# SanPen/CSparse3

Hardware: AMD Instinct MI355X
Metric: numeric-LU + lsolve/usolve nnz/s on 50k power-grid Jacobian (higher is better)
Workload: dtype f64; 1 GPU; configs[2]: synthetic banded power-grid Jacobian 50000x50000, 501330 nnz, LU refactor + 1-RHS solve per step, one matrix per GPU; n=50000, nnz_a=501330, nnz_l=696852, nnz_u=696852, rhs=1, supernodes=5970, levels=12, max_front=469, ordering=amd(A+A')

## Files before the change

csparse3_amd/csrc/cs3_internal.hpp:

```cpp
#pragma once
#include <cstdint>
#include <string>
#include <vector>

#include "../../include/csparse3_amd.h"

namespace cs3 {

using i32 = int32_t;
using i64 = int64_t;

void set_error(const std::string &msg);

void symmetrized_pattern(i64 n, const i32 *Ap, const i32 *Ai,
                         std::vector<i64> &Cp, std::vector<i32> &Ci);
void amd_order(i64 n, const std::vector<i64> &Cp, const std::vector<i32> &Ci,
               std::vector<i32> &perm);

i64 match_scale(i64 n, const i32 *Ap, const i32 *Ai, const double *Ax, i32 *rowperm, double *dr, double *dc);

void etree_upper(i64 n, const i32 *Ap, const i32 *Ai, i32 *parent);
void tree_postorder(i64 n, const i32 *parent, i32 *post);
void cholesky_counts(i64 n, const i32 *Ap, const i32 *Ai, const i32 *parent,
                     const i32 *post, i32 *colcount);

enum FrontClass : int { FC_R16 = 0, FC_R32 = 1, FC_R64 = 2, FC_LDS = 3, FC_BIG = 4, FC_IL = 5, FC_SUB = 6, FC_COUNT = 7 };

enum SolveKind : int {
    SK_SMALL = 0,
    SK_WAVE = 1,
    SK_BLOCK = 2,
    SK_BIG = 3,
    SK_IL = 4,
    SK_SUB = 5
};

struct LaunchGroup {
    int level;
    int cls;
    i32 first, count;
    i32 max_r;
    i32 max_w;
    i32 n16 = 0;
};

constexpr i32 SUB_RMAX = 32;

struct SubFront {
    i32 lpan, upan;
    i32 cb;
    i32 cv;
    i32 c0, r, w;
    i32 a_begin, a_count;
    i32 child_begin, child_count;
    i32 rel;
    i32 st;
    i32 u_sj;
    i32 parent;
    i32 arena;
};

struct SubTask {
    i32 front0, nfronts;
    i32 lvl0, nlevels;
    i32 rel0, nrel;
    i32 child0, nchild;
};

struct SubForest {
    i32 ntasks = 0;
    i32 max_fronts = 0, max_levels = 0, max_rel = 0, max_child = 0;
    i32 max_arena = 0;
    i32 max_varena = 0;
    i32 max_r = 0;
    bool empty() const { return ntasks == 0; }
};
// ... 86 lines not shown
```

csparse3_amd/csrc/kernels.hip:

```cpp
#include <hip/hip_runtime.h>


#include <stdint.h>

#include <algorithm>
#include <cstdlib>

#include "cs3_device.hpp"
#include "cs3_devfn.hpp"

namespace cs3 {

hipError_t set_withhold_handover(int on)
{
    hipError_t e = hipMemcpyToSymbol(HIP_SYMBOL(g_withhold_handover), &on, sizeof(int));
    return e != hipSuccess ? e : set_withhold_handover_forest(on);
}

typedef double double4_t __attribute__((ext_vector_type(4)));

__device__ __forceinline__ double *il_lane_base(const IlView &il, long long m)
{
    return il.base + (m >> 6) * 64 * il.len + (m & 63);
}
// ... 1141 lines not shown
{
    const long long t_start = tbuf ? (long long) __builtin_amdgcn_s_memtime() : 0;
#define CS3_BSTAMP(p) do { if (tbuf && kb == 64 && blockIdx.x == 1 && blockIdx.y == 0 && threadIdx.x == 0) \
        tbuf[(long long) (first + blockIdx.z / batch) * 8 + (p)] = (long long) __builtin_amdgcn_s_memtime() - t_start; } while (0)
#define CS3_BSTAMP_ROW(p) do { if (tbuf && kb == 64 && blockIdx.x == 0 && blockIdx.y == 1 && threadIdx.x == 0) \
        tbuf[(long long) (first + blockIdx.z / batch) * 8 + (p)] = (long long) __builtin_amdgcn_s_memtime() - t_start; } while (0)
    __shared__ double As[BIG_NB][64 + 1];
    __shared__ double Bs[BIG_NB][64 + 1];
    __shared__ double Ad[BIG_NB][BIG_NB + 1];
    __shared__ double Bd[BIG_NB][BIG_NB + 1];
    __shared__ double D[BIG_NB][BIG_NB + 1];
    __shared__ double T[64][BIG_NB + 1];
    __shared__ int pair_ready[2];
    if (threadIdx.x < 2) pair_ready[threadIdx.x] = 0;
    const FrontDesc d = fdesc[first + blockIdx.z / batch];
    const int bz = blockIdx.z % batch;
    const int r = d.r, w = d.w;
    const int nblk = (w + BIG_NB - 1) / BIG_NB;
    if (kb > nblk * BIG_NB) return;
    const bool has_panel = kb < w;
    const int ke = has_panel ? min(kb + BIG_NB, w) : w, bw = ke - kb;
    const int kp = kb - BIG_NB, pw = min(kb, w) - kp;
    double *F = pool_all + (long long) bz * pool_stride + d.lpan;
    double *dbuf = dbuf_all + (long long) bz * dbuf_stride + d.dbuf;
    const long long ld = r;
    const int tid = threadIdx.x;
    const int bi = blockIdx.x, bj = blockIdx.y;
    const int nsl = (r - ke + 63) / 64;
    if (bi > nsl || bj > nsl) return;
    if (KIND == CS3_CHOLESKY && bi < bj) return;
    if (kb > 0 && bi == 0 && bj == 0) {
        const int blk = kb / BIG_NB - 1;
        const int k0 = blk * BIG_NB, cw = min(BIG_NB, w - k0);
        for (int e = tid; e < cw * cw; e += 256) {
            const int i = e % cw, j = e / cw;
            if (KIND == CS3_LU || i >= j) F[(k0 + i) + (k0 + j) * ld] = dbuf[blk * (BIG_NB * BIG_NB) + i + j * BIG_NB];
        }
    }
    if (!has_panel && (bi == 0 || bj == 0)) return;
    const int row0 = (bi == 0) ? kb : ke + (bi - 1) * 64, nrow = (bi == 0) ? bw : min(64, r - row0);
    const int col0 = (bj == 0) ? kb : ke + (bj - 1) * 64, ncol = (bj == 0) ? bw : min(64, r - col0);
    const bool needs_d = has_panel && (bi == 0 || bj == 0);

    auto raw = [](const double *__restrict__ p, long long off, bool ok) -> double { return p[ok ? off : 0]; };
    double ra[8], rb[8], rad[4], rbd[4];
    if (kb > 0) {
#pragma unroll
        for (int q = 0; q < 8; ++q) {
            const int e = tid + 256 * q;
            { const int i = e % 64, k = e / 64; ra[q] = raw(F, (row0 + i) + (long long) (kp + k) * ld, k < pw && i < nrow); }
            if (KIND == CS3_LU) { const int k = e % BIG_NB, j = e / BIG_NB; rb[q] = raw(F, (kp + k) + (long long) (col0 + j) * ld, k < pw && j < ncol); }
            else { const int j = e % 64, k = e / 64; rb[q] = raw(F, (col0 + j) + (long long) (kp + k) * ld, k < pw && j < ncol); }
        }
#pragma unroll
        for (int q = 0; q < 4; ++q) {
            const int e = tid + 256 * q;
            { const int i = e % BIG_NB, k = e / BIG_NB; rad[q] = raw(F, (kb + i) + (long long) (kp + k) * ld, needs_d && k < pw && i < bw); }
            if (KIND == CS3_LU) { const int k = e % BIG_NB, j = e / BIG_NB; rbd[q] = raw(F, (kp + k) + (long long) (kb + j) * ld, needs_d && k < pw && j < bw); }
            else { const int j = e % BIG_NB, k = e / BIG_NB; rbd[q] = raw(F, (kb + j) + (long long) (kp + k) * ld, needs_d && k < pw && j < bw); }
        }
    }
    const int wv = tid >> 6, mi = tid & 15, mq = (tid >> 4) & 3;
    const int ti = 16 * wv + mi;
    double4_t acc[4];
#pragma unroll
    for (int cb = 0; cb < 4; ++cb)
#pragma unroll
// ... 71 lines not shown
        D[dr][j] = (dr < bw && j < bw) ? dacc[v] : (dr == j ? 1.0 : 0.0);
    }
    if (bi > 0) {
#pragma unroll
        for (int cb = 0; cb < 2; ++cb)
#pragma unroll
            for (int v = 0; v < 4; ++v) T[ti][16 * cb + mq + 4 * v] = acc[cb][v];
    } else if (bj > 0 && wv < 2) {
#pragma unroll
        for (int cb = 0; cb < 4; ++cb)
#pragma unroll
            for (int v = 0; v < 4; ++v) T[16 * cb + mq + 4 * v][ti] = acc[cb][v];
    }
    __syncthreads();
    CS3_BSTAMP(3);
    const int lane = tid & 63, half = (tid >> 6) & 1, part = tid >> 7, li = lane & 31;
    const bool stacked = lane >= 32;
    const bool row_tile = (bi == 0 && bj > 0);
    const bool diag_tile = (bi == 0 && bj == 0);
    if (diag_tile && half == 1) return;
    constexpr int HC = PAIR_NC;
    const int cbase = HC * part;
    double e[HC];
#pragma unroll
    for (int j = 0; j < HC; ++j) {
        const double dv = row_tile ? D[cbase + j][li] : D[li][cbase + j];
        const double tv = T[32 * half + li][cbase + j];
        e[j] = stacked ? (diag_tile ? 0.0 : tv) : dv;
    }
    eliminate_pair<KIND>(e, part, row_tile, (half == 0) ? &As[0][0] : &Bs[0][0], &pair_ready[half], status);
    CS3_BSTAMP(4);
    CS3_BSTAMP_ROW(6);
    if (diag_tile) {
        double *db = dbuf + (long long) (kb / BIG_NB) * (BIG_NB * BIG_NB);
        if (lane < bw) {
#pragma unroll
            for (int jj = 0; jj < HC; ++jj) {
                const int j = cbase + jj;
                if (j < bw) {
                    const double v = e[jj];
                    if (KIND == CS3_LU) {
                        if (lane > j) { if (!(fabs(v) <= inv_tol)) flag_column(status, d.c0 + kb + j); }
                        else if (lane == j) { if (!(fabs(v) > 0.0) || !(fabs(v) < 1.0e300)) flag_column(status, d.c0 + kb + j); }
                    } else if (lane == j) {
                        if (!(v > 0.0)) flag_column(status, d.c0 + kb + j);
                    }
                    db[lane + j * BIG_NB] = v;
                }
            }
        }
        return;
    }
    const int tr = 32 * half + li;
    if (stacked) {
        if (!row_tile) {
            if (tr < nrow) {
#pragma unroll
                for (int cc = 0; cc < HC; ++cc) {
                    const int c = cbase + cc;
                    if (c < bw) {
                        if (KIND == CS3_LU && !(fabs(e[cc]) <= inv_tol)) flag_column(status, d.c0 + kb + c);
                        F[(row0 + tr) + (long long) (kb + c) * ld] = e[cc];
                    }
                }
            }
        } else if (tr < ncol) {
#pragma unroll
            for (int cc = 0; cc < HC; ++cc) {
                const int c = cbase + cc;
                if (c < bw) F[(kb + c) + (long long) (col0 + tr) * ld] = e[cc];
            }
        }
    }
    CS3_BSTAMP(5);
    CS3_BSTAMP_ROW(7);
#undef CS3_BSTAMP
#undef CS3_BSTAMP_ROW
}


// ... 783 lines not shown
    const int b = blockIdx.y / nrhs, rhs = blockIdx.y % nrhs;
    const int r = d.r, w = d.w, nb = r - w;
    const double *pool = pool_all + (long long) b * pool_stride;
    const double *X = X_all + (long long) b * x_stride;
    double *v = bigv_all + ((long long) b * nrhs + rhs) * bv_size + d.bv;
    const int *st = st_idx + d.st;
    const int tid = threadIdx.x;
    for (int j = tid; j < nb; j += 256) v2[j] = X[(long long) st[w + j] * nrhs + rhs];
    __syncthreads();
    const double *L = pool + d.lpan;
    const double *U = pool + d.upan;
    for (int i = blockIdx.x * 256 + tid; i < w; i += gridDim.x * 256) {
        double acc = 0.0;
        for (int j0 = 0; j0 < nb; j0 += 16) {
            double u[16];
#pragma unroll
            for (int j = 0; j < 16; ++j) {
                const int jj = j0 + j;
                const long long off = (KIND == CS3_LU) ? (long long) i * d.u_sk + (long long) jj * d.u_sj
                                                       : (long long) (w + jj) + (long long) i * r;
                u[j] = load_if((KIND == CS3_LU) ? U : L, off, jj < nb);
            }
#pragma unroll
            for (int j = 0; j < 16; ++j) acc += u[j] * v2[j0 + j < nb ? j0 + j : 0];
        }
        v[i] = X[(long long) (d.c0 + i) * nrhs + rhs] - acc;
    }
}

template <int KIND, int CW>
__global__ void __launch_bounds__(256)
k_bwd_big_step(const SolveDesc *__restrict__ sd, int first, int chunk_from_right,
               const double *__restrict__ pool_all, double *__restrict__ X_all, double *__restrict__ bigv_all,
               int nrhs, long long pool_stride, long long x_stride, long long bv_size)
{
    constexpr int SC = CW / 4;
    __shared__ double y[BIG_CW];
    __shared__ double cpl[64];
    __shared__ double part[4][64];
    const SolveDesc d = sd[first + blockIdx.z];
    const int r = d.r, w = d.w;
    const int nchunk = (w + CW - 1) / CW;
    const int c = nchunk - 1 - chunk_from_right;
    if (c < 0) return;
    const int kb = c * CW, bw = min(CW, w - kb);
    const int bwa = min(SOLVE_BW, bw), bwb = bw - bwa;
    const int nsl = (kb + 63) / 64;
    if ((int) blockIdx.x > 0 && (int) blockIdx.x >= nsl) return;
    const int b = blockIdx.y / nrhs, rhs = blockIdx.y % nrhs;
    const double *L = pool_all + (long long) b * pool_stride + d.lpan;
    double *v = bigv_all + ((long long) b * nrhs + rhs) * bv_size + d.bv;
    const int tid = threadIdx.x, lane = tid & 63, wv = tid >> 6;
    const int row = blockIdx.x * 64 + lane;
    double us[SC];
#pragma unroll
    for (int j = 0; j < SC; ++j) {
        const int jj = wv * SC + j;
        const long long off = (KIND == CS3_LU) ? (long long) row + (long long) (kb + jj) * r
                                               : (long long) (kb + jj) + (long long) row * r;
        us[j] = load_if(L, off, row < kb && jj < bw);
    }
    if (wv == 0) {
        if (bwb > 0) {
            BlockTriangle<KIND, false> tb;
            tb.load(L, r, kb + SOLVE_BW, bwb);
            const double vi = tb.solve(load_if(v, kb + SOLVE_BW + lane, lane < bwb), bwb);
            if (lane < bwb) y[SOLVE_BW + lane] = vi;
        }
        __syncthreads();
        __syncthreads();
    } else if (wv == 1) {
        BlockTriangle<KIND, false> ta;
        ta.load(L, r, kb, bwa);
        __syncthreads();
        __syncthreads();
        const double vi = ta.solve(cpl[lane], bwa);
        if (lane < bwa) y[lane] = vi;
    } else if (wv == 2) {
        double tm[SOLVE_BW];
#pragma unroll
        for (int j = 0; j < SOLVE_BW; ++j) {
            const long long i = kb + lane, k = kb + SOLVE_BW + j;
            const long long off = (KIND == CS3_LU) ? i + k * r : k + i * r;
            tm[j] = load_if(L, off, lane < bwa && j < bwb);
        }
        double vi = load_if(v, kb + lane, lane < bwa);
        __syncthreads();
#pragma unroll
        for (int j = 0; j < SOLVE_BW; ++j) vi -= tm[j] * ((j < bwb) ? y[SOLVE_BW + j] : 0.0);
        cpl[lane] = vi;
        __syncthreads();
    } else {
        __syncthreads();
        __syncthreads();
    }
    __syncthreads();
    if (blockIdx.x == 0 && tid < bw)
        X_all[(long long) b * x_stride + (long long) (d.c0 + kb + tid) * nrhs + rhs] = y[tid];
    double acc = 0.0;
#pragma unroll
    for (int j = 0; j < SC; ++j) {
        const int jj = wv * SC + j;
        acc += us[j] * y[jj < bw ? jj : 0];
    }
    part[wv][lane] = acc;
    __syncthreads();
    if (tid < 64 && row < kb)
        v[row] -= ((part[0][tid] + part[1][tid]) + part[2][tid]) + part[3][tid];
}

constexpr int IL_KB = 4;
constexpr int IL_T = 8;
constexpr int IL_TJ = 4;
constexpr int IL_NONE = INT32_MIN;
constexpr int IL_AV = 32;

template <int KIND>
__global__ void __launch_bounds__(64)
k_front_il(const FrontDesc *__restrict__ fdesc, int first, const int *__restrict__ pairs,
           const double *__restrict__ ax_all, long long nnz_a, IlView il,
           const double *__restrict__ pool_pm_all, long long pm_stride, int batch, double inv_tol, int *status)
{
    const FrontDesc d = fdesc[first + blockIdx.x];
    const int lane = threadIdx.x;
    const long long m = (long long) blockIdx.y * 64 + lane;
    const bool live = m < batch;
    const long long mm = live ? m : (long long) blockIdx.y * 64;
    double *G = il.base + (long long) blockIdx.y * 64 * il.len + lane;
    const double *P = pool_pm_all + mm * pm_stride;
    const double *ax = ax_all + mm * nnz_a;
    const int r = d.r, w = d.w;
    double *F = G + d.lpan * 64;
#define EL(i, j) F[((long long) (i) + (long long) (j) * r) * 64]

    {
        const int np = d.a_count;
        const int *pr = pairs + 2 * d.a_begin;
        int cur = -1;
        double acc = 0.0;
        int ptg_n = pr[2 * (lane < min(64, np) ? lane : 0)], psr_n = pr[2 * (lane < min(64, np) ? lane : 0) + 1];
        for (int base = 0; base < np; base += 64) {
// ... 868 lines not shown

__global__ void __launch_bounds__(256)
k_restack_values(long long nnz, const int *__restrict__ map, long long na, long long nb, long long nc,
                 const double *__restrict__ Ax, const double *__restrict__ Bx, const double *__restrict__ Cx,
                 const double *__restrict__ Dx, double *__restrict__ Px)
{
    for (long long p = (long long) blockIdx.x * blockDim.x + threadIdx.x; p < nnz; p += (long long) gridDim.x * blockDim.x) {
        const long long s = map[p];
        Px[p] = (s < na) ? Ax[s] : (s < na + nb) ? Bx[s - na] : (s < na + nb + nc) ? Cx[s - na - nb] : Dx[s - na - nb - nc];
    }
}

hipError_t launch_restack_values(long long nnz, const int *map, long long na, long long nb, long long nc, const double *Ax,
                                 const double *Bx, const double *Cx, const double *Dx, double *Px, hipStream_t st)
{
    if (nnz == 0) return hipSuccess;
    hipLaunchKernelGGL(k_restack_values, dim3((unsigned) std::min<long long>((nnz + 255) / 256, 4096)), dim3(256), 0, st, nnz, map,
                       na, nb, nc, Ax, Bx, Cx, Dx, Px);
    return hipGetLastError();
}

constexpr int RHS_LANES_MIN = 16;
#define CS3_LAUNCH_CHECK() do { hipError_t e_ = hipGetLastError(); if (e_ != hipSuccess) return e_; } while (0)

static int grid_for(long long work, int block, int cap = 4096)
{
    long long g = (work + block - 1) / block;
    if (g < 1) g = 1;
    if (g > cap) g = cap;
    return (int) g;
}

static int big_group_blocks(const LaunchGroup &g) { return (g.max_w + BIG_NB - 1) / BIG_NB; }

static hipError_t launch_big_gather(const DeviceFactor &D, const LaunchGroup &g, hipStream_t st)
{
    const int gx = std::max(1, std::min(64, (g.max_r + 7) / 8));
    hipLaunchKernelGGL(k_big_gather, dim3(gx, (unsigned) D.batch, g.count), dim3(256), 0, st, D.fdesc, g.first, D.kind,
                       AsmLists{D.fa_tgt, D.fa_src, D.ch_tab, D.rel_idx}, D.ax, D.pool_pm, D.nnz_a, D.pm_stride, IlView{D.pool_il, D.il_len});
    CS3_LAUNCH_CHECK();
    return hipSuccess;
}

template <int KIND>
static hipError_t launch_big_block(const DeviceFactor &D, const LaunchGroup &g, int blk, double inv_tol, hipStream_t st)
{
    const unsigned batch = (unsigned) D.batch;
    const int kb = blk * BIG_NB;
    const int start = std::max(1, kb - BIG_NB + 1);
    const int rem = g.max_r - std::min(start, g.max_r);
    const int tiles = 1 + (rem + 63) / 64;
    hipLaunchKernelGGL((k_big_step<KIND>), dim3(tiles, tiles, g.count * batch), dim3(256), 0, st, D.fdesc,
                       g.first, kb, D.pool_pm, D.pm_stride, D.dbuf, D.dbuf_size, inv_tol, D.status, (int) batch, D.tbuf);
    CS3_LAUNCH_CHECK();
    return hipSuccess;
}

static int wg_panel_ld(const LaunchGroup &g) { return (g.max_r + 1) | 1; }
constexpr int WG_NB = 16;
static int wg_nb() { return WG_NB; }
static size_t wg_lds_bytes(int kind, const LaunchGroup &g)
{
    return ((size_t) wg_nb() * 33 + (size_t) (kind == CS3_LU ? 2 : 1) * wg_nb() * wg_panel_ld(g) +
            (kind == CS3_LU ? 0 : (size_t) 16 * (size_t) g.max_w)) * sizeof(double);
}
bool big_group_in_one_workgroup(int kind, long long batch, const LaunchGroup &g)
{
    static const long long min_batch = getenv("CS3_WG_MIN_BATCH") ? atoll(getenv("CS3_WG_MIN_BATCH")) : 48;
    return g.cls == FC_BIG && batch >= min_batch && wg_lds_bytes(kind, g) <= 150 * 1024;
}

template <int KIND>
static hipError_t launch_front_group(const DeviceFactor &D, const SweepCall &call, const LaunchGroup &g, double inv_tol, hipStream_t st)
{
    const unsigned batch = (unsigned) D.batch;
    if (g.cls == FC_SUB) return launch_sub_factor(D, call, inv_tol, st);
    if (big_group_in_one_workgroup(KIND, D.batch, g)) {
        hipLaunchKernelGGL((k_front_wg<KIND, WG_NB>), dim3((unsigned) g.count, batch), dim3(512), wg_lds_bytes(KIND, g), st, D.fdesc,
                           g.first, AsmLists{D.fa_tgt, D.fa_src, D.ch_tab, D.rel_idx}, D.ax, D.pool_pm, D.nnz_a, D.pm_stride,
                           IlView{D.pool_il, D.il_len}, inv_tol, D.status, wg_panel_ld(g), D.tbuf);
        CS3_LAUNCH_CHECK();
        return hipSuccess;
    }
    if (g.cls == FC_IL) {
        hipLaunchKernelGGL((k_front_il<KIND>), dim3((unsigned) g.count, (unsigned) D.ngroups), dim3(64), 0, st, D.fdesc, g.first,
                           D.ila_pairs, D.ax, D.nnz_a, IlView{D.pool_il, D.il_len}, D.pool_pm, D.pm_stride, (int) D.batch,
                           inv_tol, D.status);
        CS3_LAUNCH_CHECK();
        return hipSuccess;
    }
    if (g.cls == FC_BIG) {
        hipError_t e = launch_big_gather(D, g, st);
        for (int blk = 0; e == hipSuccess && blk <= big_group_blocks(g); ++blk) e = launch_big_block<KIND>(D, g, blk, inv_tol, st);
        return e;
    }
    dim3 grid((unsigned) g.count, batch);
    const size_t ld = (size_t) (g.max_r | 1);
    const bool packed = KIND == CS3_CHOLESKY && g.max_w <= 32;
    const size_t lds = ((packed ? (size_t) g.max_r * (size_t) (g.max_r + 1) / 2 : ld * (size_t) g.max_r) + 4 * (size_t) g.max_r + 6) * sizeof(double);
#define CS3_FRONT_ARGS D.fdesc, g.first, AsmLists{D.fa_tgt, D.fa_src, D.ch_tab, D.rel_idx}, D.ax, D.pool_pm, D.nnz_a, D.pm_stride, IlView{D.pool_il, D.il_len}, inv_tol, D.status, D.tbuf
    switch (g.cls) {
    case FC_R16:
    case FC_R32:
        hipLaunchKernelGGL((k_front_wave<KIND>), grid, dim3(64), lds, st, CS3_FRONT_ARGS); break;
    case FC_R64: {
        const unsigned threads = (D.batch >= 16 && g.max_w <= 32) ? 128 : 256;
        hipLaunchKernelGGL((k_front_mix<KIND>), grid, dim3(threads), lds, st, CS3_FRONT_ARGS); break;
    }
    default:
        const size_t blds = ((KIND == CS3_LU) ? ld * (size_t) g.max_r : (size_t) g.max_r * (size_t) (g.max_r + 1) / 2) * sizeof(double) + 16;
        if (KIND == CS3_CHOLESKY && D.batch >= 16)
            hipLaunchKernelGGL((k_front_block<CS3_CHOLESKY, 16, 4>), grid, dim3(256), blds, st, CS3_FRONT_ARGS);
        else
            hipLaunchKernelGGL((k_front_block<KIND, 16>), grid, dim3(512), blds, st, CS3_FRONT_ARGS);
        break;
    }
#undef CS3_FRONT_ARGS
    CS3_LAUNCH_CHECK();
    return hipSuccess;
}

__global__ void __launch_bounds__(256) k_poison_lds(int words)
{
    extern __shared__ __attribute__((aligned(16))) double pz[];
    for (int i = threadIdx.x; i < words; i += 256) pz[i] = __longlong_as_double(0x7ff8dead0000beefll);
    __syncthreads();
// ... 148 lines not shown
    pl.nchunk = (g.max_w + pl.cw - 1) / pl.cw;
    pl.slices = std::max(1, (g.max_r + 63) / 64);
    return pl;
}

static hipError_t launch_fwd_big_pre(const DeviceFactor &D, const SweepCall &call, const LaunchGroup &g, double *X, int nrhs, hipStream_t st)
{
    const BigSweepPlan pl = big_sweep_plan(D, g, nrhs);
    hipLaunchKernelGGL(k_fwd_big_gather, dim3(1, pl.by, g.count), dim3(256), 0, st, call.sd, g.first, D.fasm_src,
                       D.fasm_tgt, D.flong_src, D.cv, X, D.bigv, nrhs, D.cv_size * (long long) nrhs, D.n * (long long) nrhs, D.bv_size);
    CS3_LAUNCH_CHECK();
    return hipSuccess;
}

template <int KIND>
static hipError_t launch_fwd_big_chunk(const DeviceFactor &D, const SweepCall &call, const LaunchGroup &g, double *X, int nrhs, int c,
                                       hipStream_t st)
{
    const BigSweepPlan pl = big_sweep_plan(D, g, nrhs);
    const long long xs = D.n * (long long) nrhs, cvs = D.cv_size * (long long) nrhs;
    if (pl.wide)
        hipLaunchKernelGGL((k_fwd_big_step<KIND, BIG_CW>), dim3(pl.slices, pl.by, g.count), dim3(256), 0, st, call.sd,
                           g.first, c * pl.cw, D.pool_pm, D.cv, X, D.bigv, nrhs, D.pm_stride, cvs, xs, D.bv_size);
    else if (pl.multi)
        hipLaunchKernelGGL((k_fwd_big_step_multi<KIND>), dim3(pl.slices, pl.by_multi, g.count), dim3(256), 0, st, call.sd,
                           g.first, c * pl.cw, D.pool_pm, D.cv, X, D.bigv, nrhs, D.pm_stride, cvs, xs, D.bv_size);
    else
        hipLaunchKernelGGL((k_fwd_big_step<KIND, SOLVE_BW>), dim3(pl.slices, pl.by, g.count), dim3(256), 0, st, call.sd,
                           g.first, c * pl.cw, D.pool_pm, D.cv, X, D.bigv, nrhs, D.pm_stride, cvs, xs, D.bv_size);
    CS3_LAUNCH_CHECK();
    return hipSuccess;
}

template <int KIND>
static hipError_t launch_bwd_big_pre(const DeviceFactor &D, const SweepCall &call, const LaunchGroup &g, double *X, int nrhs, hipStream_t st)
{
    const BigSweepPlan pl = big_sweep_plan(D, g, nrhs);
    const size_t lds = (size_t) std::max(1, g.max_r) * sizeof(double);
    hipLaunchKernelGGL((k_bwd_big_init<KIND>), dim3(2, pl.by, g.count), dim3(256), lds, st, call.sd, g.first,
                       D.st_idx, D.pool_pm, X, D.bigv, nrhs, D.pm_stride, D.n * (long long) nrhs, D.bv_size);
    CS3_LAUNCH_CHECK();
    return hipSuccess;
}

template <int KIND>
static hipError_t launch_bwd_big_chunk(const DeviceFactor &D, const SweepCall &call, const LaunchGroup &g, double *X, int nrhs, int c,
                                       hipStream_t st)
{
    const BigSweepPlan pl = big_sweep_plan(D, g, nrhs);
    const long long xs = D.n * (long long) nrhs;
    if (pl.wide)
        hipLaunchKernelGGL((k_bwd_big_step<KIND, BIG_CW>), dim3(pl.slices, pl.by, g.count), dim3(256), 0, st, call.sd,
                           g.first, c, D.pool_pm, X, D.bigv, nrhs, D.pm_stride, xs, D.bv_size);
    else if (pl.multi)
        hipLaunchKernelGGL((k_bwd_big_step_multi<KIND>), dim3(pl.slices, pl.by_multi, g.count), dim3(256), 0, st, call.sd,
                           g.first, c, D.pool_pm, X, D.bigv, nrhs, D.pm_stride, xs, D.bv_size);
    else
        hipLaunchKernelGGL((k_bwd_big_step<KIND, SOLVE_BW>), dim3(pl.slices, pl.by, g.count), dim3(256), 0, st, call.sd,
                           g.first, c, D.pool_pm, X, D.bigv, nrhs, D.pm_stride, xs, D.bv_size);
    CS3_LAUNCH_CHECK();
    return hipSuccess;
}


template <int KIND>
static hipError_t launch_inv_tasks(const DeviceFactor &D, int t0, int t1, hipStream_t st)
{
    if (t1 <= t0) return hipSuccess;
    hipLaunchKernelGGL((k_inv_diag<KIND>), dim3((unsigned) (t1 - t0), (unsigned) D.batch), dim3(256), 0, st, D.sdesc, D.inv_tasks, t0,
                       D.pool_pm, D.pm_stride, D.dinv, D.dinv_size);
    CS3_LAUNCH_CHECK();
    return hipSuccess;
}

static bool gemm_sweeps_on()
{
    static const bool on = !(getenv("CS3_NO_GEMM_SWEEPS") && getenv("CS3_NO_GEMM_SWEEPS")[0] == '1');
    return on;
}

bool permutation_can_fuse(const DeviceFactor &D, int nrhs)
{
    constexpr int min_rhs = 256;
    return gemm_sweeps_on() && nrhs >= std::max(min_rhs, RHS_LANES_MIN) && D.il_len == 0;
}

hipError_t launch_diag_inverses(const DeviceFactor &D, hipStream_t st)
{
    return with_kind(D.kind, [&](auto K) { return launch_inv_tasks<K>(D, 0, D.n_inv_tasks, st); });
}

template <int KIND>
// ... 106 lines not shown
                                   D.pool_pm, X, nrhs, D.pm_stride, xs);
        }
    } else if (g.cls == SK_BIG) {
        const BigSweepPlan pl = big_sweep_plan(D, g, nrhs);
        hipError_t e = forward ? launch_fwd_big_pre(D, call, g, X, nrhs, st) : launch_bwd_big_pre<KIND>(D, call, g, X, nrhs, st);
        for (int c = 0; e == hipSuccess && c < pl.nchunk; ++c)
            e = forward ? launch_fwd_big_chunk<KIND>(D, call, g, X, nrhs, c, st) : launch_bwd_big_chunk<KIND>(D, call, g, X, nrhs, c, st);
        return e;
    } else {
        dim3 grid((unsigned) g.count, (unsigned) D.batch, (unsigned) nrhs);
        const size_t lds = (size_t) (g.max_r + 1 + SOLVE_BW) * sizeof(double);
        if (forward)
            hipLaunchKernelGGL((k_fwd_blk<KIND>), grid, dim3(256), lds, st, call.sd, g.first, D.fasm_src,
                               D.fasm_tgt, D.flong_src, D.pool_pm, D.cv, X, nrhs, D.pm_stride, cvs, xs);
        else
            hipLaunchKernelGGL((k_bwd_blk<KIND>), grid, dim3(256), lds, st, call.sd, g.first, D.st_idx,
                               D.pool_pm, X, nrhs, D.pm_stride, xs);
    }
    CS3_LAUNCH_CHECK();
    return hipSuccess;
}

static int promote_max()
{
    return 16;
}

static void absorb_small_group(std::vector<LaunchGroup> &out, const LaunchGroup &g, int small_cls, int wg_cls)
{
    if (!out.empty() && out.back().level == g.level && out.back().cls == small_cls && g.cls == wg_cls &&
        out.back().count <= promote_max() && out.back().first + out.back().count == g.first) {
        LaunchGroup &m = out.back();
        m.cls = wg_cls; m.count += g.count;
        m.max_r = std::max(m.max_r, g.max_r); m.max_w = std::max(m.max_w, g.max_w);
        m.n16 = 0;
    } else {
        out.push_back(g);
    }
}

static std::vector<LaunchGroup> sweep_groups(const std::vector<LaunchGroup> &groups, int nrhs, long long batch)
{
    if (nrhs >= RHS_LANES_MIN) return groups;
    std::vector<LaunchGroup> merged, out;
    for (const LaunchGroup &g : groups) {
        if (!merged.empty() && merged.back().level == g.level && merged.back().cls == SK_SMALL && g.cls == SK_WAVE &&
            merged.back().first + merged.back().count == g.first) {
            LaunchGroup &m = merged.back();
            m.cls = SK_WAVE; m.count += g.count;
            m.max_r = std::max(m.max_r, g.max_r); m.max_w = std::max(m.max_w, g.max_w);
        } else {
            merged.push_back(g);
        }
    }
    if (batch != 1) return merged;
    for (const LaunchGroup &g : merged) absorb_small_group(out, g, SK_WAVE, SK_BLOCK);
    return out;
}

static std::vector<LaunchGroup> factor_groups(const DeviceFactor &D, const std::vector<LaunchGroup> &groups)
{
    if (D.batch != 1) return groups;
    std::vector<LaunchGroup> out;
    for (const LaunchGroup &g : groups) absorb_small_group(out, g, FC_R64, FC_LDS);
    return out;
}

hipError_t launch_solve_levels(const DeviceFactor &D, const SweepCall &call, double *X, int nrhs, bool forward, hipStream_t st, ForkJoin &fj)
{
    const std::vector<LaunchGroup> groups = sweep_groups(*call.groups, nrhs, D.batch);
    fj.rewind();
    const bool solve_parallel = nrhs >= 512;
    auto launch = [&](const LaunchGroup &g, hipStream_t s) {
        return with_sweep_kind(D.kind, call.trans, [&](auto K) { return launch_solve_group<K>(D, call, g, X, nrhs, forward, s); });
    };
    if (forward) {
        for (size_t g0 = 0; g0 < groups.size(); ) {
            const size_t g1 = level_edge(groups, g0, true);
            hipError_t e = run_level(groups, g0, g1, st, fj, solve_parallel, launch);
            if (e != hipSuccess) return e;
            g0 = g1;
        }
    } else {
// ... 63 lines not shown
            const int level = fgroups[f0].level;
            const size_t f1 = level_edge(fgroups, f0, true);
            e = run_level(fgroups, f0, f1, st, fj, true, [&](const LaunchGroup &g, hipStream_t s2) {
                return with_kind(D.kind, [&](auto K) { return launch_front_group<K>(D, call, g, inv_tol, s2); });
            });
            if (e != hipSuccess) return e;
            if ((e = flush()) != hipSuccess) return e;
            if ((e = fj.event(&pending)) != hipSuccess) return e;
            if ((e = hipEventRecord(pending, st)) != hipSuccess) return e;
            pending_level = level;
            f0 = f1;
        }
        if ((e = flush()) != hipSuccess) return e;
        hipEvent_t done;
        if ((e = fj.event(&done)) != hipSuccess) return e;
        if ((e = hipEventRecord(done, fj.aux)) != hipSuccess) return e;
        return hipStreamWaitEvent(st, done, 0);
    }
    const LaunchGroup *rootf = nullptr, *roots = nullptr;
    if (nrhs < RHS_LANES_MIN && nlevels >= 2 && fork_level == nlevels - 2) {
        int nf = 0, ns = 0;
        for (const LaunchGroup &g : fgroups) if (g.level == nlevels - 1) { ++nf; rootf = &g; }
        for (const LaunchGroup &g : sgroups) if (g.level == nlevels - 1) { ++ns; roots = &g; }
        if (nf != 1 || ns != 1 || rootf->cls != FC_BIG || roots->cls != SK_BIG || rootf->count != roots->count)
            rootf = roots = nullptr;
    }
    hipEvent_t swept = nullptr, ready_deferred = nullptr;
    int root_rest = 0;
    for (size_t f0 = 0; f0 < fgroups.size(); ) {
        const int level = fgroups[f0].level;
        const size_t f1 = level_edge(fgroups, f0, true);
        if (rootf && level == nlevels - 1) {
            const BigSweepPlan pl = big_sweep_plan(D, *roots, nrhs);
            const int nblk = big_group_blocks(*rootf), cwb = pl.cw / BIG_NB;
            if ((e = launch_big_gather(D, *rootf, st)) != hipSuccess) return e;
            int k = 0;
            while (k < pl.nchunk && (k + 1) * cwb <= nblk && nblk - (k + 1) * cwb >= k + 2) ++k;
            hipEvent_t home = nullptr;
            bool side_started = false;
            auto start_side = [&]() -> hipError_t {
                side_started = true;
                if (ready_deferred) {
                    hipError_t se;
                    if ((se = hipStreamWaitEvent(fj.aux, ready_deferred, 0)) != hipSuccess) return se;
                    if ((se = sweep(0, fork_level, fj.aux)) != hipSuccess) return se;
                }
                return launch_fwd_big_pre(D, call, *roots, X, nrhs, fj.aux);
            };
            auto release = [&]() -> hipError_t {
                hipError_t se;
                if ((se = hipStreamWaitEvent(fj.aux, home, 0)) != hipSuccess) return se;
                for (int c = 0; c < k; ++c) {
                    se = with_sweep_kind(D.kind, call.trans,
                                         [&](auto K) { return launch_fwd_big_chunk<K>(D, call, *roots, X, nrhs, c, fj.aux); });
                    if (se != hipSuccess) return se;
                }
                home = nullptr;
                return hipSuccess;
            };
            for (int blk = 0; blk <= nblk; ++blk) {
                e = with_kind(D.kind, [&](auto K) { return launch_big_block<K>(D, *rootf, blk, inv_tol, st); });
                if (e != hipSuccess) return e;
                if (!side_started && (e = start_side()) != hipSuccess) return e;
                if (home && (e = release()) != hipSuccess) return e;
                if (k > 0 && blk == k * cwb) {
                    if ((e = fj.event(&home)) != hipSuccess) return e;
                    if ((e = hipEventRecord(home, st)) != hipSuccess) return e;
                }
            }
            if (home && (e = release()) != hipSuccess) return e;
            root_rest = k;
            if ((e = fj.event(&swept)) != hipSuccess) return e;
            if ((e = hipEventRecord(swept, fj.aux)) != hipSuccess) return e;
            f0 = f1;
            continue;
        }
        e = run_level(fgroups, f0, f1, st, fj, true, [&](const LaunchGroup &g, hipStream_t s) {
            return with_kind(D.kind, [&](auto K) { return launch_front_group<K>(D, call, g, inv_tol, s); });
        });
        if (e != hipSuccess) return e;
        if (ready_deferred && !rootf) {
            if ((e = hipStreamWaitEvent(fj.aux, ready_deferred, 0)) != hipSuccess) return e;
            if ((e = sweep(0, fork_level, fj.aux)) != hipSuccess) return e;
            if ((e = fj.event(&swept)) != hipSuccess) return e;
            if ((e = hipEventRecord(swept, fj.aux)) != hipSuccess) return e;
            ready_deferred = nullptr;
        }
        if (level == fork_level) {
            hipEvent_t ready;
            if ((e = fj.event(&ready)) != hipSuccess) return e;
            if ((e = hipEventRecord(ready, st)) != hipSuccess) return e;
            ready_deferred = ready;
        }
// ... 68 lines not shown
```

csparse3_amd/csrc/symbolic.cpp:

```cpp
#include <algorithm>
#include <chrono>
#include <cstdlib>
#include <numeric>
#include <stdexcept>

#include "cs3_internal.hpp"
#include <cstdio>
#include <cstdlib>

namespace cs3 {

void etree_upper(i64 n, const i32 *Ap, const i32 *Ai, i32 *parent)
{
    std::vector<i32> anc(n, -1);
    for (i64 k = 0; k < n; ++k) {
        parent[k] = -1;
        for (i64 p = Ap[k]; p < Ap[k + 1]; ++p) {
            for (i32 i = Ai[p]; i != -1 && i < k; ) {
                i32 up = anc[i];
                anc[i] = (i32) k;
                if (up == -1) parent[i] = (i32) k;
                i = up;
            }
        }
// ... 738 lines not shown
            {
                const i64 r = order_r(s);
                size_t a = 0;
                for (i64 tj = 0; tj < r; ++tj)
                    for (i64 ti = (kind == CS3_CHOLESKY ? tj : 0); ti < r; ++ti) {
                        const i32 t = (i32) (ti + tj * r);
                        if (a < items.size() && items[a].tgt < t) throw std::runtime_error("analyze: source outside the stored part of a front");
                        if (a == items.size() || items[a].tgt != t) { S.ila_pairs.push_back(t); S.ila_pairs.push_back(IL_ZERO); }
                        for (; a < items.size() && items[a].tgt == t; ++a) { S.ila_pairs.push_back(t); S.ila_pairs.push_back(items[a].src); }
                    }
                if (a != items.size()) throw std::runtime_error("analyze: source outside the stored part of a front");
                while ((S.ila_pairs.size() / 2) % 16) { S.ila_pairs.push_back(-1); S.ila_pairs.push_back(IL_ZERO); }
            }
            S.ila_ptr[s + 1] = (i64) (S.ila_pairs.size() / 2);
        }
    }
    if (has_forest) fill_forest(S, fa_ptr, fa_item);

    tick("9. assembly lists");
    S.sched.resize(ns);
    std::iota(S.sched.begin(), S.sched.end(), 0);
    std::stable_sort(S.sched.begin(), S.sched.end(), [&](i32 a, i32 b) {
        if (S.sn_tlevel[a] != S.sn_tlevel[b]) return S.sn_tlevel[a] < S.sn_tlevel[b];
        return S.sn_class[a] < S.sn_class[b];
    });
    S.groups.clear();
    for (i32 t = 0; t < ns; ) {
        i32 s = S.sched[t];
        LaunchGroup g{S.sn_tlevel[s], S.sn_class[s], t, 0, 0, 0, 0};
        while (t < ns && S.sn_tlevel[S.sched[t]] == g.level && S.sn_class[S.sched[t]] == g.cls) {
            const i32 f = S.sched[t];
            g.max_r = std::max<i32>(g.max_r, (i32) order_r(f));
            g.max_w = std::max<i32>(g.max_w, (i32) width(f));
            ++t;
        }
        g.count = t - g.first;
        S.groups.push_back(g);
    }
    tick("10. launch groups");
    std::vector<i32> cs_count;
    std::vector<Item> cs_out;
    auto sort_by_row = [&](std::vector<Item> &items, i64 r) {
        cs_count.assign((size_t) r + 1, 0);
        for (const Item &it : items) ++cs_count[(size_t) it.tgt + 1];
        for (i64 t = 0; t < r; ++t) cs_count[(size_t) t + 1] += cs_count[(size_t) t];
        cs_out.resize(items.size());
        for (const Item &it : items) cs_out[(size_t) cs_count[(size_t) it.tgt]++] = it;
        items.swap(cs_out);
    };
    S.fasm_ptr.assign(ns + 1, 0);
    S.fasm_src.clear(); S.fasm_tgt.clear(); S.flong_src.clear();
    {
        std::vector<Item> items;
        for (i32 s = 0; s < ns; ++s) {
            items.clear();
            const i64 w = width(s);
            for (i64 i = 0; i < w; ++i) items.push_back(Item{(i32) i, (i32) ~(S.sn_ptr[s] + i)});
            for (i32 cp = S.child_ptr[s]; cp < S.child_ptr[s + 1]; ++cp) {
                const i32 c = S.child_idx[cp];
                const i64 nbc = order_r(c) - width(c);
                const i32 *rel = S.rel_idx.data() + S.rel_ptr[c];
                for (i64 ii = 0; ii < nbc; ++ii) items.push_back(Item{rel[ii], (i32) (S.cv_off[c] + ii)});
            }
            sort_by_row(items, order_r(s));
            emit_runs(items, S.fasm_tgt, S.fasm_src, S.flong_src);
            S.fasm_ptr[s + 1] = (i64) S.fasm_tgt.size();
// ... 42 lines not shown
                for (const Item &it : items) S.sl_src[base + (size_t) (fill[(size_t) it.tgt]++ * stride + it.tgt)] = it.src;
                S.sl_rounds[s] = rounds;
            }
            S.rl_ptr[s + 1] = (i64) (S.rl_pairs.size() / 2);
            S.sl_ptr[s + 1] = (i64) S.sl_src.size();
        }
    }
    S.ssched.resize(ns);
    std::iota(S.ssched.begin(), S.ssched.end(), 0);
    std::stable_sort(S.ssched.begin(), S.ssched.end(), [&](i32 a, i32 b) {
        if (S.sn_level[a] != S.sn_level[b]) return S.sn_level[a] < S.sn_level[b];
        if (solve_kind(a) != solve_kind(b)) return solve_kind(a) < solve_kind(b);
        return (order_r(a) <= 16) > (order_r(b) <= 16);
    });
    S.gv_off.assign(ns, 0); S.dinv_off.assign(ns, 0); S.gv_size = 0; S.dinv_size = 0; S.inv_tasks.clear();
    for (i32 t = 0; t < ns; ++t) {
        const i32 s = S.ssched[t];
        const int sk = solve_kind(s);
        if (sk != SK_WAVE && sk != SK_BLOCK && sk != SK_BIG) continue;
        S.gv_off[s] = S.gv_size; S.gv_size += order_r(s);
        S.dinv_off[s] = S.dinv_size;
        const i64 nchunk = (width(s) + 63) / 64;
        S.dinv_size += nchunk * 2 * 4096;
        for (i64 c = 0; c < nchunk; ++c) { S.inv_tasks.push_back(t); S.inv_tasks.push_back((i32) c); }
    }
    S.sgroups.clear();
    for (i32 t = 0; t < ns; ) {
        i32 s = S.ssched[t];
        LaunchGroup g{S.sn_level[s], solve_kind(s), t, 0, 0, 0, 0};
        while (t < ns && S.sn_level[S.ssched[t]] == g.level && solve_kind(S.ssched[t]) == g.cls) {
            const i32 f = S.ssched[t];
            g.max_r = std::max<i32>(g.max_r, (i32) order_r(f));
            g.max_w = std::max<i32>(g.max_w, (i32) width(f));
            if (order_r(f) <= 16) ++g.n16;
            ++t;
        }
        g.count = t - g.first;
        S.sgroups.push_back(g);
    }

    S.ssched1.clear(); S.sgroups1.clear();
    if (has_forest) {
        auto kind1 = [&](i32 s) { return in_forest(s) ? (int) SK_SUB : solve_kind(s); };
        S.ssched1.resize(ns);
        std::iota(S.ssched1.begin(), S.ssched1.end(), 0);
        std::stable_sort(S.ssched1.begin(), S.ssched1.end(), [&](i32 a, i32 b) {
            if (S.sn_tlevel[a] != S.sn_tlevel[b]) return S.sn_tlevel[a] < S.sn_tlevel[b];
            return kind1(a) < kind1(b);
        });
        for (i32 t = 0; t < ns; ) {
            i32 s = S.ssched1[t];
            LaunchGroup g{S.sn_tlevel[s], kind1(s), t, 0, 0, 0, 0};
            while (t < ns && S.sn_tlevel[S.ssched1[t]] == g.level && kind1(S.ssched1[t]) == g.cls) {
                const i32 f = S.ssched1[t];
                g.max_r = std::max<i32>(g.max_r, (i32) order_r(f));
                g.max_w = std::max<i32>(g.max_w, (i32) width(f));
                ++t;
            }
            g.count = t - g.first;
            S.sgroups1.push_back(g);
        }
    }

    if (getenv("CS3_DUMP_GROUPS")) {
        for (const LaunchGroup &g : S.groups)
            fprintf(stderr, "factor level %2d cls %d count %6d max_r %4d max_w %4d\n", g.level, g.cls, g.count, g.max_r, g.max_w);
        for (const LaunchGroup &g : S.sgroups)
            fprintf(stderr, "solve  level %2d kind %d count %6d max_r %4d max_w %4d\n", g.level, g.cls, g.count, g.max_r, g.max_w);
        for (const LaunchGroup &g : S.sgroups1)
            fprintf(stderr, "solve1 level %2d kind %d count %6d max_r %4d max_w %4d\n", g.level, g.cls, g.count, g.max_r, g.max_w);
        const SubForest &T = S.sub_forest;
        if (!T.empty())
            fprintf(stderr, "forest: %d tasks, max fronts %d levels %d rel %d child %d arena %d max_r %d\n", T.ntasks, T.max_fronts,
                    T.max_levels, T.max_rel, T.max_child, T.max_arena, T.max_r);
    }

    tick("10b. sweep lists and schedules");
    S.nnz_l = 0;
    for (i64 j = 0; j < n; ++j) S.nnz_l += S.colcount[j];
    S.nnz_u = (kind == CS3_LU) ? S.nnz_l : 0;
    S.Lp.clear(); S.Li.clear(); S.Up.clear(); S.Ui.clear(); S.Lmap.clear(); S.Umap.clear();
    S.t_symbolic = seconds_since(t0);
}


void build_csc_factors(Symbolic &S)
{
    if (!S.Lp.empty() || S.n == 0) { if (S.n == 0 && S.Lp.empty()) { S.Lp.assign(1, 0); if (S.kind == CS3_LU) S.Up.assign(1, 0); } return; }
    const i64 n = S.n;
// ... 121 lines not shown
```

Before: 4.472 billion nnz/s.

## Skip trailing big-front launch and bwd init pass for root fronts without border

Adds a per-group max_nb (rows beyond the pivot block). When it is zero (root fronts), the diagonal tile of the last panel is written straight into the factor instead of the dbuf staging buffer, so the final copy-back launch of the big-front factorization is skipped. The backward big solve for such groups reads the RHS directly from X on its first chunk and drops the separate init kernel, parking intermediate results in the bigv buffer. This removes one kernel launch in each of the factor and solve paths on the root, at the cost of more conditional logic and branches whose correctness depends on consistent handling of the parked values.

```diff
diff --git a/csparse3_amd/csrc/cs3_internal.hpp b/csparse3_amd/csrc/cs3_internal.hpp
--- a/csparse3_amd/csrc/cs3_internal.hpp
+++ b/csparse3_amd/csrc/cs3_internal.hpp
@@ -42,6 +42,7 @@
     i32 max_r;
     i32 max_w;
     i32 n16 = 0;
+    i32 max_nb = 0;
 };
 
 constexpr i32 SUB_RMAX = 32;
diff --git a/csparse3_amd/csrc/kernels.hip b/csparse3_amd/csrc/kernels.hip
--- a/csparse3_amd/csrc/kernels.hip
+++ b/csparse3_amd/csrc/kernels.hip
@@ -1197,7 +1197,8 @@
     if (kb > 0 && bi == 0 && bj == 0) {
         const int blk = kb / BIG_NB - 1;
         const int k0 = blk * BIG_NB, cw = min(BIG_NB, w - k0);
-        for (int e = tid; e < cw * cw; e += 256) {
+        const bool parked = k0 + cw < r;
+        for (int e = tid; parked && e < cw * cw; e += 256) {
             const int i = e % cw, j = e / cw;
             if (KIND == CS3_LU || i >= j) F[(k0 + i) + (k0 + j) * ld] = dbuf[blk * (BIG_NB * BIG_NB) + i + j * BIG_NB];
         }
@@ -1335,7 +1336,9 @@
     CS3_BSTAMP(4);
     CS3_BSTAMP_ROW(6);
     if (diag_tile) {
-        double *db = dbuf + (long long) (kb / BIG_NB) * (BIG_NB * BIG_NB);
+        const bool home = ke == r;
+        double *db = home ? F + kb + kb * ld : dbuf + (long long) (kb / BIG_NB) * (BIG_NB * BIG_NB);
+        const long long dld = home ? ld : BIG_NB;
         if (lane < bw) {
 #pragma unroll
             for (int jj = 0; jj < HC; ++jj) {
@@ -1348,7 +1351,7 @@
                     } else if (lane == j) {
                         if (!(v > 0.0)) flag_column(status, d.c0 + kb + j);
                     }
-                    db[lane + j * BIG_NB] = v;
+                    if (!home || KIND == CS3_LU || lane >= j) db[lane + j * dld] = v;
                 }
             }
         }
@@ -2198,7 +2201,7 @@
 __global__ void __launch_bounds__(256)
 k_bwd_big_step(const SolveDesc *__restrict__ sd, int first, int chunk_from_right,
                const double *__restrict__ pool_all, double *__restrict__ X_all, double *__restrict__ bigv_all,
-               int nrhs, long long pool_stride, long long x_stride, long long bv_size)
+               int nrhs, long long pool_stride, long long x_stride, long long bv_size, int from_x)
 {
     constexpr int SC = CW / 4;
     __shared__ double y[BIG_CW];
@@ -2216,8 +2219,18 @@
     const int b = blockIdx.y / nrhs, rhs = blockIdx.y % nrhs;
     const double *L = pool_all + (long long) b * pool_stride + d.lpan;
     double *v = bigv_all + ((long long) b * nrhs + rhs) * bv_size + d.bv;
+    double *Xf = X_all + (long long) b * x_stride + (long long) d.c0 * nrhs + rhs;
+    const bool first_from_x = from_x && chunk_from_right == 0;
+    const bool park = first_from_x && c > 0;
     const int tid = threadIdx.x, lane = tid & 63, wv = tid >> 6;
     const int row = blockIdx.x * 64 + lane;
+    auto rhs_row = [&](int i, bool ok) -> double {
+        return first_from_x ? load_if(Xf, (long long) i * nrhs, ok) : load_if(v, i, ok);
+    };
+    if (from_x && chunk_from_right == 1 && blockIdx.x == 0) {
+        const int pk = kb + CW, pw = min(CW, w - pk);
+        if (tid < pw) Xf[(long long) (pk + tid) * nrhs] = v[pk + tid];
+    }
     double us[SC];
 #pragma unroll
     for (int j = 0; j < SC; ++j) {
@@ -2230,7 +2243,7 @@
         if (bwb > 0) {
             BlockTriangle<KIND, false> tb;
             tb.load(L, r, kb + SOLVE_BW, bwb);
-            const double vi = tb.solve(load_if(v, kb + SOLVE_BW + lane, lane < bwb), bwb);
+            const double vi = tb.solve(rhs_row(kb + SOLVE_BW + lane, lane < bwb), bwb);
             if (lane < bwb) y[SOLVE_BW + lane] = vi;
         }
         __syncthreads();
@@ -2250,7 +2263,7 @@
             const long long off = (KIND == CS3_LU) ? i + k * r : k + i * r;
             tm[j] = load_if(L, off, lane < bwa && j < bwb);
         }
-        double vi = load_if(v, kb + lane, lane < bwa);
+        double vi = rhs_row(kb + lane, lane < bwa);
         __syncthreads();
 #pragma unroll
         for (int j = 0; j < SOLVE_BW; ++j) vi -= tm[j] * ((j < bwb) ? y[SOLVE_BW + j] : 0.0);
@@ -2261,8 +2274,10 @@
         __syncthreads();
     }
     __syncthreads();
-    if (blockIdx.x == 0 && tid < bw)
-        X_all[(long long) b * x_stride + (long long) (d.c0 + kb + tid) * nrhs + rhs] = y[tid];
+    if (blockIdx.x == 0 && tid < bw) {
+        if (park) v[kb + tid] = y[tid];
+        else Xf[(long long) (kb + tid) * nrhs] = y[tid];
+    }
     double acc = 0.0;
 #pragma unroll
     for (int j = 0; j < SC; ++j) {
@@ -2272,7 +2287,7 @@
     part[wv][lane] = acc;
     __syncthreads();
     if (tid < 64 && row < kb)
-        v[row] -= ((part[0][tid] + part[1][tid]) + part[2][tid]) + part[3][tid];
+        v[row] = rhs_row(row, true) - (((part[0][tid] + part[1][tid]) + part[2][tid]) + part[3][tid]);
 }
 
 constexpr int IL_KB = 4;
@@ -3207,6 +3222,7 @@
 }
 
 static int big_group_blocks(const LaunchGroup &g) { return (g.max_w + BIG_NB - 1) / BIG_NB; }
+static int big_group_last_launch(const LaunchGroup &g) { return big_group_blocks(g) - (g.max_nb == 0 ? 1 : 0); }
 
 static hipError_t launch_big_gather(const DeviceFactor &D, const LaunchGroup &g, hipStream_t st)
 {
@@ -3266,7 +3282,7 @@
     }
     if (g.cls == FC_BIG) {
         hipError_t e = launch_big_gather(D, g, st);
-        for (int blk = 0; e == hipSuccess && blk <= big_group_blocks(g); ++blk) e = launch_big_block<KIND>(D, g, blk, inv_tol, st);
+        for (int blk = 0; e == hipSuccess && blk <= big_group_last_launch(g); ++blk) e = launch_big_block<KIND>(D, g, blk, inv_tol, st);
         return e;
     }
     dim3 grid((unsigned) g.count, batch);
@@ -3481,10 +3497,13 @@
     return hipSuccess;
 }
 
+static bool bwd_big_from_x(const BigSweepPlan &pl, const LaunchGroup &g) { return g.max_nb == 0 && (pl.wide || !pl.multi); }
+
 template <int KIND>
 static hipError_t launch_bwd_big_pre(const DeviceFactor &D, const SweepCall &call, const LaunchGroup &g, double *X, int nrhs, hipStream_t st)
 {
     const BigSweepPlan pl = big_sweep_plan(D, g, nrhs);
+    if (bwd_big_from_x(pl, g)) return hipSuccess;
     const size_t lds = (size_t) std::max(1, g.max_r) * sizeof(double);
     hipLaunchKernelGGL((k_bwd_big_init<KIND>), dim3(2, pl.by, g.count), dim3(256), lds, st, call.sd, g.first,
                        D.st_idx, D.pool_pm, X, D.bigv, nrhs, D.pm_stride, D.n * (long long) nrhs, D.bv_size);
@@ -3500,13 +3519,13 @@
     const long long xs = D.n * (long long) nrhs;
     if (pl.wide)
         hipLaunchKernelGGL((k_bwd_big_step<KIND, BIG_CW>), dim3(pl.slices, pl.by, g.count), dim3(256), 0, st, call.sd,
-                           g.first, c, D.pool_pm, X, D.bigv, nrhs, D.pm_stride, xs, D.bv_size);
+                           g.first, c, D.pool_pm, X, D.bigv, nrhs, D.pm_stride, xs, D.bv_size, bwd_big_from_x(pl, g) ? 1 : 0);
     else if (pl.multi)
         hipLaunchKernelGGL((k_bwd_big_step_multi<KIND>), dim3(pl.slices, pl.by_multi, g.count), dim3(256), 0, st, call.sd,
                            g.first, c, D.pool_pm, X, D.bigv, nrhs, D.pm_stride, xs, D.bv_size);
     else
         hipLaunchKernelGGL((k_bwd_big_step<KIND, SOLVE_BW>), dim3(pl.slices, pl.by, g.count), dim3(256), 0, st, call.sd,
-                           g.first, c, D.pool_pm, X, D.bigv, nrhs, D.pm_stride, xs, D.bv_size);
+                           g.first, c, D.pool_pm, X, D.bigv, nrhs, D.pm_stride, xs, D.bv_size, bwd_big_from_x(pl, g) ? 1 : 0);
     CS3_LAUNCH_CHECK();
     return hipSuccess;
 }
@@ -3679,7 +3698,7 @@
         out.back().count <= promote_max() && out.back().first + out.back().count == g.first) {
         LaunchGroup &m = out.back();
         m.cls = wg_cls; m.count += g.count;
-        m.max_r = std::max(m.max_r, g.max_r); m.max_w = std::max(m.max_w, g.max_w);
+        m.max_r = std::max(m.max_r, g.max_r); m.max_w = std::max(m.max_w, g.max_w); m.max_nb = std::max(m.max_nb, g.max_nb);
         m.n16 = 0;
     } else {
         out.push_back(g);
@@ -3695,7 +3714,7 @@
             merged.back().first + merged.back().count == g.first) {
             LaunchGroup &m = merged.back();
             m.cls = SK_WAVE; m.count += g.count;
-            m.max_r = std::max(m.max_r, g.max_r); m.max_w = std::max(m.max_w, g.max_w);
+            m.max_r = std::max(m.max_r, g.max_r); m.max_w = std::max(m.max_w, g.max_w); m.max_nb = std::max(m.max_nb, g.max_nb);
         } else {
             merged.push_back(g);
         }
@@ -3825,10 +3844,10 @@
         const size_t f1 = level_edge(fgroups, f0, true);
         if (rootf && level == nlevels - 1) {
             const BigSweepPlan pl = big_sweep_plan(D, *roots, nrhs);
-            const int nblk = big_group_blocks(*rootf), cwb = pl.cw / BIG_NB;
+            const int nblk = big_group_blocks(*rootf), last = big_group_last_launch(*rootf), cwb = pl.cw / BIG_NB;
             if ((e = launch_big_gather(D, *rootf, st)) != hipSuccess) return e;
             int k = 0;
-            while (k < pl.nchunk && (k + 1) * cwb <= nblk && nblk - (k + 1) * cwb >= k + 2) ++k;
+            while (k < pl.nchunk && (k + 1) * cwb <= nblk && last - (k + 1) * cwb >= k + 2) ++k;
             hipEvent_t home = nullptr;
             bool side_started = false;
             auto start_side = [&]() -> hipError_t {
@@ -3851,7 +3870,7 @@
                 home = nullptr;
                 return hipSuccess;
             };
-            for (int blk = 0; blk <= nblk; ++blk) {
+            for (int blk = 0; blk <= last; ++blk) {
                 e = with_kind(D.kind, [&](auto K) { return launch_big_block<K>(D, *rootf, blk, inv_tol, st); });
                 if (e != hipSuccess) return e;
                 if (!side_started && (e = start_side()) != hipSuccess) return e;
diff --git a/csparse3_amd/csrc/symbolic.cpp b/csparse3_amd/csrc/symbolic.cpp
--- a/csparse3_amd/csrc/symbolic.cpp
+++ b/csparse3_amd/csrc/symbolic.cpp
@@ -794,6 +794,7 @@
             const i32 f = S.sched[t];
             g.max_r = std::max<i32>(g.max_r, (i32) order_r(f));
             g.max_w = std::max<i32>(g.max_w, (i32) width(f));
+            g.max_nb = std::max<i32>(g.max_nb, (i32) (order_r(f) - width(f)));
             ++t;
         }
         g.count = t - g.first;
@@ -902,6 +903,7 @@
             const i32 f = S.ssched[t];
             g.max_r = std::max<i32>(g.max_r, (i32) order_r(f));
             g.max_w = std::max<i32>(g.max_w, (i32) width(f));
+            g.max_nb = std::max<i32>(g.max_nb, (i32) (order_r(f) - width(f)));
             if (order_r(f) <= 16) ++g.n16;
             ++t;
         }
@@ -925,6 +927,7 @@
                 const i32 f = S.ssched1[t];
                 g.max_r = std::max<i32>(g.max_r, (i32) order_r(f));
                 g.max_w = std::max<i32>(g.max_w, (i32) width(f));
+                g.max_nb = std::max<i32>(g.max_nb, (i32) (order_r(f) - width(f)));
                 ++t;
             }
             g.count = t - g.first;
```

Measured after the change: 4.517 billion nnz/s, median of 6. No clear change (+1.0%).
